# rodluger/starry_process

Hardware: AMD Instinct MI355X
Metric: log_likelihood evals/sec (ydeg=15, K=1000) (higher is better)
Workload: dtype f64

## Files before the change

starry_process_amd/csrc/sp_cov.h:

```cpp
#ifndef SP_COV_H
#define SP_COV_H

#include "sp_internal.h"

__device__ __forceinline__ int star_nobs(const sp_star &st, int K) {
  return (st.nobs > 0 && st.nobs < K) ? st.nobs : K;
}

__device__ __forceinline__ double temporal_factor(int kind, double ti, double tj,
                                                  double tau) {
#pragma clang fp contract(off)
  if (kind == SP_TEMPORAL_NONE) return 1.0;
  const double dt = fabs(ti - tj);
  if (kind == SP_TEMPORAL_MATERN32) {
    const double x = 1.7320508075688772 * dt / tau;
    return (1.0 + x) * exp(-x);
  }
  return exp(-(dt * dt) / (2.0 * tau));
}

__device__ __forceinline__ double temporal_dfactor_dtau(int kind, double ti, double tj,
                                                        double tau) {
  if (kind == SP_TEMPORAL_NONE) return 0.0;
  const double dt = fabs(ti - tj);
  if (kind == SP_TEMPORAL_MATERN32) {
    const double x = 1.7320508075688772 * dt / tau;
    return x * x / tau * exp(-x);
  }
  return (dt * dt) / (2.0 * tau * tau) * exp(-(dt * dt) / (2.0 * tau));
}

template <int CTRL>
__device__ __forceinline__ double dpp_move(double v) {
  const int lo = __builtin_amdgcn_mov_dpp(__double2loint(v), CTRL, 0xf, 0xf, true);
  const int hi = __builtin_amdgcn_mov_dpp(__double2hiint(v), CTRL, 0xf, 0xf, true);
  return __hiloint2double(hi, lo);
}
template <int N>
__device__ __forceinline__ void row16_sum(double (&x)[N]) {
#pragma unroll
  for (int k = 0; k < N; ++k) x[k] += dpp_move<0xB1>(x[k]);
#pragma unroll
  for (int k = 0; k < N; ++k) x[k] += dpp_move<0x4E>(x[k]);
#pragma unroll
  for (int k = 0; k < N; ++k) x[k] += dpp_move<0x141>(x[k]);
#pragma unroll
  for (int k = 0; k < N; ++k) x[k] += dpp_move<0x140>(x[k]);
}

typedef double dd2 __attribute__((ext_vector_type(2)));

struct SplineGen {
  const double *tab;
  int np2;
  double dx, inv_dx;
  int covpts;
  __device__ __forceinline__ double operator()(double thi, double thj) const {
#pragma clang fp contract(off)
    const double x = fabs(thi - thj);
    const double q = x * inv_dx;
    int idx = (int)q;
    double x0 = q - (double)idx;
    if (fabs(x0 - 0.5) > 0.5 - 1.0e-9) {
      idx = (int)floor(x / dx);
      x0 = q - (double)idx;
    }
    idx = idx > covpts ? covpts : idx;
    typedef const __attribute__((address_space(3))) dd2 *lds_dd2;
    const unsigned a1 = (unsigned)(size_t)(const __attribute__((address_space(3))) double *)tab + ((unsigned)idx << 4);
    const dd2 c01 = *(lds_dd2)(size_t)a1;
    const dd2 c23 = *(lds_dd2)(size_t)(a1 + 8u * (unsigned)np2);
    return __builtin_fma(x0, __builtin_fma(x0, __builtin_fma(x0, c23.y, c23.x), c01.y), c01.x);
  }
  template <int N>
  __device__ __forceinline__ void many(const double (&thi)[N], const double (&thj)[N], double (&out)[N]) const {
#pragma clang fp contract(off)
    double x0[N];
    int idx[N];
    bool odd = false;
#pragma unroll
    for (int e = 0; e < N; ++e) {
      const double q = fabs(thi[e] - thj[e]) * inv_dx;
      idx[e] = (int)q;
      x0[e] = q - (double)idx[e];
      odd |= fabs(x0[e] - 0.5) > 0.5 - 1.0e-9;
    }
    if (__builtin_expect(odd, 0)) {
#pragma unroll
      for (int e = 0; e < N; ++e)
        if (fabs(x0[e] - 0.5) > 0.5 - 1.0e-9) {
          const double x = fabs(thi[e] - thj[e]);
          idx[e] = (int)floor(x / dx);
          x0[e] = x * inv_dx - (double)idx[e];
        }
    }
    dd2 c01[N], c23[N];
    typedef const __attribute__((address_space(3))) dd2 *lds_dd2;
    const unsigned base = (unsigned)(size_t)(const __attribute__((address_space(3))) double *)tab;
    const unsigned off2 = 8u * (unsigned)np2;
#pragma unroll
    for (int e = 0; e < N; ++e) {
      const int k = idx[e] > covpts ? covpts : idx[e];
      const unsigned a1 = base + ((unsigned)k << 4);
      c01[e] = *(lds_dd2)(size_t)a1;
      c23[e] = *(lds_dd2)(size_t)(a1 + off2);
    }
#pragma unroll
    for (int e = 0; e < N; ++e)
      out[e] = __builtin_fma(x0[e], __builtin_fma(x0[e], __builtin_fma(x0[e], c23[e].y, c23[e].x), c01[e].y), c01[e].x);
  }
};


__device__ __forceinline__ void spline_table_to_lds(const double *__restrict__ src, double *stage, int np, int tid) {
  const int n2 = 2 * np;
  dd2 v[4];
#pragma unroll
  for (int c = 0; c < 4; ++c) {
    const int e = tid + 256 * c;
    v[c] = e < n2 ? *reinterpret_cast<const dd2 *>(src + 2 * e) : dd2{0.0, 0.0};
  }
#pragma unroll
  for (int c = 0; c < 4; ++c) {
    const int e = tid + 256 * c;
    if (e < n2) *reinterpret_cast<dd2 *>(stage + 2 * e) = v[c];
  }
  for (int e = tid + 1024; e < n2; e += 256)
    *reinterpret_cast<dd2 *>(stage + 2 * e) = *reinterpret_cast<const dd2 *>(src + 2 * e);
}


#ifndef SP_LAZY_BATCH
#define SP_LAZY_BATCH 8
#endif
template <int MA, typename V4>
__device__ __forceinline__ void lazy_cov_tiles(const LazyCov &z, int star, const int (&ri)[MA][4],
                                               const int (&cj)[4], V4 (&out)[MA][4], double *stage) {
  const sp_star st = z.stars[star];
  const int nobs = star_nobs(st, z.K), np = z.covpts + 4;
  const double *th = z.theta + (size_t)star * z.K, *tt = z.t + (size_t)star * z.K;
  const bool tk = z.temporal != SP_TEMPORAL_NONE;
#ifdef SP_LAZY_NO_SEP
  const bool sep = false;
#else
  const bool sep = z.temporal == SP_TEMPORAL_MATERN32 && z.inorder && z.inorder[star] != 0.0;
#endif
  double thi[MA][4], ti[MA][4], thj[4], tj[4];
#pragma unroll
  for (int k = 0; k < 4; ++k) {
    const bool oj = cj[k] < nobs;
    thj[k] = oj ? th[cj[k]] : 0.0;
    tj[k] = (oj && tk) ? tt[cj[k]] : 0.0;
#pragma unroll
    for (int m = 0; m < MA; ++m) {
      const bool oi = ri[m][k] < nobs;
      thi[m][k] = oi ? th[ri[m][k]] : 0.0;
      ti[m][k] = (oi && tk) ? tt[ri[m][k]] : 0.0;
    }
  }
  const int c0 = cj[0] & ~63;
  const double tb = sep ? tt[c0 < nobs ? c0 : nobs - 1] : 0.0;
  spline_table_to_lds(z.ptab + (size_t)star * 4 * np, stage, np, threadIdx.x);
  __syncthreads();
  SplineGen g{stage, 2 * np, 6.283185307179586 / z.covpts,
              1.0 / (6.283185307179586 / z.covpts), z.covpts};
  const double cm = sep ? 1.7320508075688772 / st.tau : 0.0;
  double fc[4] = {1.0, 1.0, 1.0, 1.0};
  bool fok[4] = {false, false, false, false};
  if (sep) {
#pragma unroll
    for (int n = 0; n < 4; ++n) {
      const double a = cm * (tj[n] - tb);
      fok[n] = a < 600.0 && a >= 0.0;
      fc[n] = exp(fok[n] ? a : 0.0);
    }
  }
#pragma unroll
  for (int m = 0; m < MA; ++m) {
    double er[4] = {1.0, 1.0, 1.0, 1.0};
    if (sep) {
#pragma unroll
      for (int r = 0; r < 4; ++r) er[r] = exp(-(cm * (ti[m][r] - tb)));
    }
#pragma unroll
    for (int n0 = 0; n0 < 4; n0 += SP_LAZY_BATCH / 4) {
      double a[SP_LAZY_BATCH], b[SP_LAZY_BATCH], v[SP_LAZY_BATCH];
#pragma unroll
      for (int e = 0; e < SP_LAZY_BATCH; ++e) {
        a[e] = thi[m][e & 3];
        b[e] = thj[n0 + (e >> 2)];
      }
      g.many<SP_LAZY_BATCH>(a, b, v);
#pragma unroll
      for (int e = 0; e < SP_LAZY_BATCH; ++e) {
        const int n = n0 + (e >> 2), r = e & 3;
        double w = 0.0;
        if (ri[m][r] < nobs && cj[n] < nobs) {
#pragma clang fp contract(off)
          if (sep && fok[n]) {
            const double x = cm * (ti[m][r] - tj[n]);
            w = v[e] * ((1.0 + x) * (er[r] * fc[n]));
          } else {
            w = v[e] * temporal_factor(z.temporal, ti[m][r], tj[n], st.tau);
          }
        }
        out[m][n][r] = w;
      }
    }
    if (z.rid) {
#pragma unroll
      for (int r = 0; r < 4; ++r) {
        const int mr = ri[m][r] - z.K;
        if (mr < 0 || mr >= z.nrid) continue;
        const double *src = z.rid + ((size_t)star * (z.nrid + 1) + mr) * z.K;
        double x[4];
#pragma unroll
        for (int n = 0; n < 4; ++n) x[n] = src[cj[n] < z.K ? cj[n] : z.K - 1];
#pragma unroll
        for (int n = 0; n < 4; ++n) out[m][n][r] = cj[n] < z.K ? x[n] : 0.0;
      }
    }
  }
  __syncthreads();
}

template <typename V4>
__device__ __forceinline__ void lazy_diag_block(const LazyCov &z, int star, const SplineGen &g, const sp_star &st,
                                                int nobs, const int (&ri)[4], int cj, V4 &out) {
  const double *th = z.theta + (size_t)star * z.K, *tt = z.t + (size_t)star * z.K;
  const double *rb = z.rid + (size_t)star * (z.nrid + 1) * z.K;
  const bool tk = z.temporal != SP_TEMPORAL_NONE;
  const int cc = cj < z.K ? cj : z.K - 1;
  const double thj = th[cc], tj = tk ? tt[cc] : 0.0;
  double thi[4], ti[4], dd[4], rv[4];
#pragma unroll
  for (int r = 0; r < 4; ++r) {
    const int rc = ri[r] < z.K ? ri[r] : z.K - 1;
    thi[r] = th[rc];
    ti[r] = tk ? tt[rc] : 0.0;
    dd[r] = rb[(size_t)z.nrid * z.K + rc];
    const int m = ri[r] - z.K;
    rv[r] = rb[(size_t)((m >= 0 && m < z.nrid) ? m : 0) * z.K + cc];
  }
#pragma unroll
  for (int r = 0; r < 4; ++r) {
    const int m = ri[r] - z.K;
    double v;
    if (ri[r] < nobs && cj < nobs) {
#pragma clang fp contract(off)
      v = g(thi[r], thj) * temporal_factor(z.temporal, ti[r], tj, st.tau);
      if (ri[r] == cj) v += dd[r];
    } else if (m >= 0 && m < z.nrid && cj < z.K) {
      v = rv[r];
    } else {
      v = ri[r] == cj ? 1.0 : 0.0;
    }
    out[r] = v;
  }
}

#ifndef SP_LAZY_ROW_BATCH
#define SP_LAZY_ROW_BATCH 0
#endif
template <int ROWB, typename V4>
__device__ __forceinline__ void lazy_cov_row(const LazyCov &z, int star, int ri, int c0, V4 (&out)[4],
                                             double *stage, int tid) {
  const sp_star st = z.stars[star];
  const int nobs = star_nobs(st, z.K), np = z.covpts + 4;
  const double *th = z.theta + (size_t)star * z.K;
  const bool oi = ri < nobs;
  const double thi = oi ? th[ri] : 0.0;
  double *s_thj = stage + 4 * np;
  {
    const double *src = z.ptab + (size_t)star * 4 * np;
    const int n2 = 2 * np, cbase = c0 & ~63;
    dd2 v[3];
#pragma unroll
    for (int c = 0; c < 3; ++c) {
      const int e = tid + 256 * c;
      v[c] = e < n2 ? *reinterpret_cast<const dd2 *>(src + 2 * e) : dd2{0.0, 0.0};
    }
    const double tj = (tid < 64 && cbase + tid < nobs) ? th[cbase + tid] : 0.0;
#pragma unroll
    for (int c = 0; c < 3; ++c) {
      const int e = tid + 256 * c;
      if (e < n2) *reinterpret_cast<dd2 *>(stage + 2 * e) = v[c];
    }
    for (int e = tid + 768; e < n2; e += 256)
      *reinterpret_cast<dd2 *>(stage + 2 * e) = *reinterpret_cast<const dd2 *>(src + 2 * e);
    if (tid < 64) s_thj[tid] = tj;
  }
  __syncthreads();
  SplineGen g{stage, 2 * np, 6.283185307179586 / z.covpts,
              1.0 / (6.283185307179586 / z.covpts), z.covpts};
  const int cl = c0 & 63;
  if constexpr (ROWB == 2) {
#pragma unroll
  for (int m = 0; m < 4; ++m) {
    V4 o;
#pragma unroll
    for (int half = 0; half < 2; ++half) {
      const dd2 tt = *reinterpret_cast<const dd2 *>(s_thj + cl + 16 * m + 2 * half);
      const double a[2] = {thi, thi}, b[2] = {tt.x, tt.y};
      double v[2];
      g.many<2>(a, b, v);
      o[2 * half] = (oi && c0 + 16 * m + 2 * half < nobs) ? v[0] : 0.0;
      o[2 * half + 1] = (oi && c0 + 16 * m + 2 * half + 1 < nobs) ? v[1] : 0.0;
      __builtin_amdgcn_sched_barrier(0);
    }
    out[m] = o;
  }
  } else if constexpr (ROWB == 0) {
#pragma unroll
  for (int m = 0; m < 4; ++m) {
    const dd2 t01 = *reinterpret_cast<const dd2 *>(s_thj + cl + 16 * m), t23 = *reinterpret_cast<const dd2 *>(s_thj + cl + 16 * m + 2);
    const double thj[4] = {t01.x, t01.y, t23.x, t23.y};
    V4 o;
#pragma unroll
    for (int r = 0; r < 4; ++r) o[r] = (oi && c0 + 16 * m + r < nobs) ? g(thi, thj[r]) : 0.0;
    out[m] = o;
  }
  } else {
#pragma unroll
  for (int m0 = 0; m0 < 4; m0 += ROWB / 4) {
    double a[ROWB], b[ROWB], v[ROWB];
#pragma unroll
    for (int h = 0; h < ROWB / 4; ++h) {
      const dd2 t01 = *reinterpret_cast<const dd2 *>(s_thj + cl + 16 * (m0 + h));
      const dd2 t23 = *reinterpret_cast<const dd2 *>(s_thj + cl + 16 * (m0 + h) + 2);
      a[4 * h] = a[4 * h + 1] = a[4 * h + 2] = a[4 * h + 3] = thi;
      b[4 * h] = t01.x;
      b[4 * h + 1] = t01.y;
      b[4 * h + 2] = t23.x;
      b[4 * h + 3] = t23.y;
    }
    g.many<ROWB>(a, b, v);
#pragma unroll
    for (int h = 0; h < ROWB / 4; ++h) {
      V4 o;
#pragma unroll
      for (int r = 0; r < 4; ++r) o[r] = (oi && c0 + 16 * (m0 + h) + r < nobs) ? v[4 * h + r] : 0.0;
      out[m0 + h] = o;
    }
    __builtin_amdgcn_sched_barrier(0);
  }
  }
  if (z.rid && !oi) {
    const int mr = ri - z.K;
    if (mr >= 0 && mr < z.nrid) {
      const double *src = z.rid + ((size_t)star * (z.nrid + 1) + mr) * z.K;
      double x[16];
#pragma unroll
      for (int e = 0; e < 16; ++e) {
        const int c = c0 + 16 * (e >> 2) + (e & 3);
        x[e] = src[c < z.K ? c : z.K - 1];
      }
#pragma unroll
      for (int m = 0; m < 4; ++m) {
        V4 o;
#pragma unroll
        for (int r = 0; r < 4; ++r) o[r] = c0 + 16 * m + r < z.K ? x[4 * m + r] : 0.0;
        out[m] = o;
      }
    }
  }
  __syncthreads();
}

#endif
```

starry_process_amd/csrc/sp_gemm.hip:

```cpp
#include <cstdlib>

#include <type_traits>

#include "sp_internal.h"
#include "sp_tile.h"
#include "sp_cov.h"
#include "sp_mm.h"
#include "sp_stage.h"
#include "sp_paneldiag.h"

typedef double d2 __attribute__((ext_vector_type(2)));

#define GT SP_GT

namespace {

__global__ __launch_bounds__(256) void gemm_nt_kernel(
    const double *A, long lda, long strideA, const double *__restrict__ B, long ldb, long strideB,
    double *C, long ldc, long strideC, int Mrows, int Nrows, int Kd, double alpha, int beta,
    int lower_only, int batch, int ntn, int ntiles, const int32_t *__restrict__ bsel, int nsel) {
  constexpr int BK = 32, LDW = BK + 1;
  __shared__ __attribute__((aligned(16))) double smem[2 * GT * LDW];
  double *sA = smem, *sB = smem + GT * LDW;
  int mtx, tile;
  if (!sp_xcd_decode(blockIdx.x, batch, ntiles, mtx, tile)) return;
  int ti, tj;
  if (lower_only) {
    ti = (int)((sqrt(8.0 * tile + 1.0) - 1.0) * 0.5);
    while (ti * (ti + 1) / 2 > tile) --ti;
    while ((ti + 1) * (ti + 2) / 2 <= tile) ++ti;
    tj = tile - ti * (ti + 1) / 2;
  } else {
    ti = tile / ntn;
    tj = tile % ntn;
  }
  const int row0 = ti * GT, col0 = tj * GT;
  const double *Ab = A + (size_t)mtx * strideA;
  int bm = mtx;
  if (bsel) {
    bm = bsel[mtx];
    if (bm < 0 || bm >= nsel) bm = 0;
  }
  const double *Bb = B + (size_t)bm * strideB;
  double *Cb = C + (size_t)mtx * strideC;
  const int lane = threadIdx.x & 63, wave = threadIdx.x >> 6;
  const int fr = lane & 15, fk = lane >> 4;
  d4 acc[4];
#pragma unroll
  for (int n = 0; n < 4; ++n) acc[n] = d4{0.0, 0.0, 0.0, 0.0};
  const bool full = row0 + GT <= Mrows && col0 + GT <= Nrows;
  if (beta) {
#pragma unroll
    for (int n = 0; n < 4; ++n)
#pragma unroll
      for (int r = 0; r < 4; ++r) {
        const int gi = row0 + 16 * wave + fk + 4 * r, gj = col0 + 16 * n + fr;
        if (full || (gi < Mrows && gj < Nrows)) acc[n][r] = Cb[(size_t)gi * ldc + gj];
      }
  }
  const bool vecA = ((lda & 1) == 0) && ((reinterpret_cast<uintptr_t>(Ab) & 15) == 0);
  const bool vecB = ((ldb & 1) == 0) && ((reinterpret_cast<uintptr_t>(Bb) & 15) == 0);
  PanelRegs<BK> ra, rb;
  if (Kd > 0) {
    stage_load<BK>(Ab, lda, row0, Mrows, 0, Kd, vecA, ra);
    stage_load<BK>(Bb, ldb, col0, Nrows, 0, Kd, vecB, rb);
  }
  for (int k0 = 0; k0 < Kd; k0 += BK) {
    stage_store<BK>(ra, alpha, sA);
    stage_store<BK>(rb, 1.0, sB);
    __syncthreads();
    if (k0 + BK < Kd) {
      stage_load<BK>(Ab, lda, row0, Mrows, k0 + BK, Kd, vecA, ra);
      stage_load<BK>(Bb, ldb, col0, Nrows, k0 + BK, Kd, vecB, rb);
    }
    const double *pa = sA + (16 * wave + fr) * LDW + fk;
    const double *pb = sB + fr * LDW + fk;
#pragma unroll
    for (int kk = 0; kk < BK; kk += 4) {
      const double a = pa[kk];
      acc[0] = __builtin_amdgcn_mfma_f64_16x16x4f64(a, pb[kk], acc[0], 0, 0, 0);
      acc[1] = __builtin_amdgcn_mfma_f64_16x16x4f64(a, pb[16 * LDW + kk], acc[1], 0, 0, 0);
      acc[2] = __builtin_amdgcn_mfma_f64_16x16x4f64(a, pb[32 * LDW + kk], acc[2], 0, 0, 0);
      acc[3] = __builtin_amdgcn_mfma_f64_16x16x4f64(a, pb[48 * LDW + kk], acc[3], 0, 0, 0);
    }
    __syncthreads();
  }
#pragma unroll
  for (int n = 0; n < 4; ++n)
#pragma unroll
    for (int r = 0; r < 4; ++r) {
      const int gi = row0 + 16 * wave + fk + 4 * r, gj = col0 + 16 * n + fr;
      if (full || (gi < Mrows && gj < Nrows)) Cb[(size_t)gi * ldc + gj] = acc[n][r];
    }
}

}

namespace {
#ifdef SP_MM_STAMPS
__device__ long long sp_mm_dbg[8 * 4096];
#endif
#ifndef SP_MM_WAVES
#define SP_MM_WAVES 1
#endif
#ifndef SP_MM_SYRK_NS
#define SP_MM_SYRK_NS 6
#endif
template <class Core, bool SGN, bool SEL = false>
__global__ __launch_bounds__(256, SP_MM_WAVES) void mm_nt_kernel(
    const double *__restrict__ A, long lda, long strideA, const double *__restrict__ B, long ldb,
    long strideB, double *__restrict__ C, long ldc, long strideC, int Kd, double alpha, int beta,
    int lower_only, int batch, int ntn, int ntiles, int skip00, LazyCov lz, DiagFuse df,
    const int32_t *__restrict__ bsel, int nsel) {
  constexpr int TM = Core::TM_, TN = Core::TN_;
  static_assert(Core::LDS_DOUBLES >= SP_DIAG_LDS_DOUBLES, "the tile-(0,0) workgroup factors a pivot block in this LDS");
  __shared__ __attribute__((aligned(16))) double lds[Core::LDS_DOUBLES];
#ifdef SP_MM_STAMPS
  const long long wall_begin = wall_clock64(), cyc_begin = __builtin_readcyclecounter();
#endif
  int mtx, tile;
  if (!sp_xcd_decode(blockIdx.x, batch, ntiles, mtx, tile)) return;
  int ti, tj;
  if (lower_only) {
    ti = (int)((sqrt(8.0 * tile + 1.0) - 1.0) * 0.5);
    while (ti * (ti + 1) / 2 > tile) --ti;
    while ((ti + 1) * (ti + 2) / 2 <= tile) ++ti;
    tj = tile - ti * (ti + 1) / 2;
  } else {
    ti = tile / ntn;
    tj = tile % ntn;
  }
  const int tj_limit = skip00 >> 8;
  int k_first = (skip00 & 2) ? ti * TM : 0;
  if (df.tri0 >= 0 && TM == 64) {
    const int r = 64 * (df.j + ti) - df.tri0, first = r > 0 ? r / 64 - df.s0 : 0;
    if (first > 0) k_first = 64 * first < Kd ? 64 * first : Kd;
  }
  if (tj_limit && tj >= tj_limit) return;
  if ((skip00 & 1) && lower_only && ti == 0 && tj == 0) {
    if (df.sys) {
      __builtin_amdgcn_s_setprio(3);
      panel_diag_item(df.sys + (size_t)mtx * df.stride, df.ld, df.j, df.nact,
                      df.img + (size_t)mtx * df.lts + sp_img_off(df.j),
                      df.info ? df.info + mtx : nullptr, lds, threadIdx.x);
    }
    return;
  }
  const double *Ab = A + (size_t)mtx * strideA + (size_t)ti * TM * lda;
  int bm = mtx;
  if constexpr (SEL) {
    bm = bsel[mtx];
    if (bm < 0 || bm >= nsel) bm = 0;
  }
  const double *Bb = B + (size_t)bm * strideB + (size_t)tj * TN * ldb;
  double *Cb = C + (size_t)mtx * strideC + (size_t)ti * TM * ldc + (size_t)tj * TN;
  Core mm;
  mm.init(Ab, lda, Bb, ldb);
  if constexpr (SGN && Core::MA == 1 && Core::NA == 4 && TM == 64 && TN == 64) {
    if ((skip00 & 4) && lower_only && ti == tj) {
      const bool dform = beta && lz.theta && (lz.dlazy & 2);
      const int lane = threadIdx.x & 63;
      sp_star dst{};
      int dnobs = 0;
      if (dform) {
        dst = lz.stars[mtx];
        dnobs = star_nobs(dst, lz.K);
        spline_table_to_lds(lz.ptab + (size_t)mtx * 4 * (lz.covpts + 4), lds, lz.covpts + 4, threadIdx.x);
        __syncthreads();
      }
      const SplineGen dg{lds, 2 * (lz.covpts + 4), 6.283185307179586 / lz.covpts, 1.0 / (6.283185307179586 / lz.covpts),
                         lz.covpts};
      if (!dform) mm.prologue(lds, k_first, Kd);
      auto run = [&](auto wtag) {
        constexpr int W = decltype(wtag)::value;
        using D = typename Core::template SymDeal<W>;
        mm_d4 a3[3];
#pragma unroll
        for (int b = 0; b < 3; ++b) {
          mm_d4 c = mm_d4{0.0, 0.0, 0.0, 0.0};
          if (b < D::NB && dform) {
            int ri[4];
#pragma unroll
            for (int r = 0; r < 4; ++r) ri[r] = 64 * (lz.tr0 + ti) + 16 * D::brow(b) + (lane >> 4) + 4 * r;
            lazy_diag_block(lz, mtx, dg, dst, dnobs, ri, 64 * (lz.tc0 + tj) + 16 * D::bcol(b) + (lane & 15), c);
          } else if (b < D::NB && beta) {
#pragma unroll
            for (int r = 0; r < 4; ++r)
              c[r] = Cb[(size_t)(16 * D::brow(b) + (lane >> 4) + 4 * r) * ldc + 16 * D::bcol(b) + (lane & 15)];
          }
          a3[b] = alpha < 0.0 ? -c : c;
        }
        if (dform) {
          __syncthreads();
          mm.prologue(lds, k_first, Kd);
        }
        mm.template sym_loop<W>(lds, k_first, Kd, a3);
#pragma unroll
        for (int b = 0; b < D::NB; ++b)
#pragma unroll
          for (int r = 0; r < 4; ++r)
            Cb[(size_t)(16 * D::brow(b) + (lane >> 4) + 4 * r) * ldc + 16 * D::bcol(b) + (lane & 15)] =
                alpha < 0.0 ? -a3[b][r] : a3[b][r];
      };
      switch (threadIdx.x >> 6) {
        case 0: run(std::integral_constant<int, 0>{}); break;
        case 1: run(std::integral_constant<int, 1>{}); break;
        case 2: run(std::integral_constant<int, 2>{}); break;
        default: run(std::integral_constant<int, 3>{}); break;
      }
      return;
    }
  }
  mm_d4 acc[Core::MA][Core::NA], cin[SGN ? 1 : Core::MA][SGN ? 1 : Core::NA];
  constexpr bool CAN_LAZY = Core::MA == 1 && Core::NA == 4 && TM == 64 && TN == 64;
  const bool lazy = CAN_LAZY && beta && lz.theta && lz.tr0 + ti > lz.tc0 + tj && lz.tc0 + tj > 0 &&
                    lz.tr0 + ti < lz.nfull;
  mm_d4 cz1[1][4];
  mm_d4 (&cz)[4] = cz1[0];
  if (!lazy) mm.prologue(lds, k_first, Kd);
  if (lazy) {
    int ri[1][4], cj[4];
#pragma unroll
    for (int k = 0; k < 4; ++k) {
      ri[0][k] = 64 * (lz.tr0 + ti) + mm.acc_row(0, k);
      cj[k] = 64 * (lz.tc0 + tj) + mm.acc_col(k < Core::NA ? k : 0);
    }
    lazy_cov_tiles<1>(lz, mtx, ri, cj, cz1, lds);
    mm.prologue(lds, k_first, Kd);
  }
#pragma unroll
  for (int m = 0; m < Core::MA; ++m)
#pragma unroll
    for (int n = 0; n < Core::NA; ++n) {
      mm_d4 c = mm_d4{0.0, 0.0, 0.0, 0.0};
      if (lazy) {
        c = cz[n & 3];
      } else if (beta) {
#pragma unroll
        for (int r = 0; r < 4; ++r) c[r] = Cb[(size_t)mm.acc_row(m, r) * ldc + mm.acc_col(n)];
      }
      if (SGN) {
        acc[m][n] = alpha < 0.0 ? -c : c;
      } else {
        acc[m][n] = mm_d4{0.0, 0.0, 0.0, 0.0};
        cin[m][n] = c;
      }
    }
#ifdef SP_MM_STAMPS
  const long long cyc_loop = __builtin_readcyclecounter();
#endif
  mm.loop(lds, k_first, Kd, acc);
#ifdef SP_MM_STAMPS
  const long long cyc_store = __builtin_readcyclecounter();
#endif
#pragma unroll
  for (int m = 0; m < Core::MA; ++m)
#pragma unroll
    for (int n = 0; n < Core::NA; ++n)
#pragma unroll
      for (int r = 0; r < 4; ++r) {
        double v;
        if (SGN)
          v = alpha < 0.0 ? -acc[m][n][r] : acc[m][n][r];
        else
          v = fma(alpha, acc[m][n][r], cin[m][n][r]);
        Cb[(size_t)mm.acc_row(m, r) * ldc + mm.acc_col(n)] = v;
      }
#ifdef SP_MM_STAMPS
  if (threadIdx.x == 0 && lower_only && df.sys && blockIdx.x < 4096) {
    long long *o = sp_mm_dbg + 8 * blockIdx.x;
    o[0] = (long long)mtx * 4096 + tile; o[1] = lazy; o[2] = wall_begin; o[3] = wall_clock64();
    o[4] = cyc_loop - cyc_begin; o[5] = cyc_store - cyc_loop; o[6] = __builtin_readcyclecounter() - cyc_store;
    o[7] = ((__builtin_amdgcn_s_getreg(20 | (0 << 6) | (31 << 11)) & 15u) << 8) | ((__builtin_amdgcn_s_getreg(4 | (0 << 6) | (31 << 11)) >> 8) & 255u);
  }
#endif
}


using Syrk128Core = MM2<128, 64, 8, 4, 4>;
#ifndef SP_SYRK128_WGS
#define SP_SYRK128_WGS 1
#endif
__global__ __launch_bounds__(256, SP_SYRK128_WGS) void syrk128_kernel(const double *__restrict__ X, long ld, long stride,
                                                      double *__restrict__ T, int Kd, int batch, int nb, int ntiles,
                                                      LazyCov lz, DiagFuse df) {
  using Core = Syrk128Core;
  static_assert(Core::LDS_DOUBLES >= SP_DIAG_LDS_DOUBLES, "the last workgroup of a star factors a pivot block in this LDS");
  static_assert(Core::MA == 2 && Core::NA == 4, "a wavefront = 32 rows of one block row");
  __shared__ __attribute__((aligned(16))) double lds[Core::LDS_DOUBLES];
  int mtx, tile;
  if (!sp_xcd_decode(blockIdx.x, batch, ntiles, mtx, tile)) return;
  if (tile == 0) {
    if (df.sys) {
      __builtin_amdgcn_s_setprio(3);
      panel_diag_item(df.sys + (size_t)mtx * df.stride, df.ld, df.j, df.nact,
                      df.img + (size_t)mtx * df.lts + sp_img_off(df.j), df.info ? df.info + mtx : nullptr, lds, threadIdx.x);
    }
    return;
  }
  tile -= 1;
  const int o = nb & 1;
  int I = (int)((sqrt((double)((o + 1) * (o + 1) + 4 * tile)) - (o + 1)) * 0.5);
  while (I * I + I * (o + 1) > tile) --I;
  while ((I + 1) * (I + 1) + (I + 1) * (o + 1) <= tile) ++I;
  const int J = tile - (I * I + I * (o + 1)), R0 = o + 2 * I;
  const double *Xb = X + (size_t)mtx * stride;
  const double *Ab = Xb + (size_t)R0 * 64 * ld, *Bb = Xb + (size_t)J * 64 * ld;
  double *Cb = T + (size_t)mtx * stride + (size_t)R0 * 64 * ld + (size_t)J * 64;
  Core mm;
  mm.init(Ab, ld, Bb, ld);
  const int R = R0 + (mm.acc_row(0, 0) >> 6);
  const bool want = R >= J && !(R == 0 && J == 0);
  const auto is_lazy = [&](int Rb) {
    return lz.theta && lz.tr0 + Rb > lz.tc0 + J && lz.tc0 + J > 0 && lz.tr0 + Rb < lz.nfull;
  };
  const bool any_lazy = is_lazy(R0) || is_lazy(R0 + 1), my_lazy = is_lazy(R);
  mm_d4 acc[Core::MA][Core::NA];
  if (any_lazy) {
    int ri[Core::MA][4], cj[4];
#pragma unroll
    for (int k = 0; k < 4; ++k) {
      cj[k] = 64 * (lz.tc0 + J) + mm.acc_col(k);
#pragma unroll
      for (int m = 0; m < Core::MA; ++m) ri[m][k] = 64 * (lz.tr0 + R0) + mm.acc_row(m, k);
    }
    lazy_cov_tiles<Core::MA>(lz, mtx, ri, cj, acc, lds);
  }
  mm.prologue(lds, 0, Kd);
#pragma unroll
  for (int m = 0; m < Core::MA; ++m)
#pragma unroll
    for (int n = 0; n < Core::NA; ++n) {
      mm_d4 c = mm_d4{0.0, 0.0, 0.0, 0.0};
      if (any_lazy && my_lazy) {
        c = acc[m][n];
      } else if (want) {
#pragma unroll
        for (int r = 0; r < 4; ++r) c[r] = Cb[(size_t)mm.acc_row(m, r) * ld + mm.acc_col(n)];
      }
      acc[m][n] = -c;
    }
  mm.loop(lds, 0, Kd, acc);
  if (!want) return;
#pragma unroll
  for (int m = 0; m < Core::MA; ++m)
#pragma unroll
    for (int n = 0; n < Core::NA; ++n)
#pragma unroll
      for (int r = 0; r < 4; ++r) Cb[(size_t)mm.acc_row(m, r) * ld + mm.acc_col(n)] = -acc[m][n][r];
}

template <class Core>
int mm_launch(const double *A, long lda, long strideA, const double *B, long ldb, long strideB,
              double *C, long ldc, long strideC, int Mrows, int Nrows, int Kd, double alpha, int beta,
              int lower_only, int batch, hipStream_t st, int skip00, const LazyCov *lazy = nullptr,
              const DiagFuse *dfp = nullptr, const int32_t *bsel = nullptr, int nsel = 0) {
  const LazyCov lz = lazy ? *lazy : LazyCov{};
  const DiagFuse df = dfp ? *dfp : DiagFuse{nullptr, 0, 0, 0, 0, nullptr, 0, nullptr, -1, 0};
  const int ntm = Mrows / Core::TM_, ntn = Nrows / Core::TN_;
  const int ntiles = lower_only ? ntm * (ntm + 1) / 2 : ntm * ntn;
  const long nblk = sp_xcd_grid(batch, ntiles);
  if (nblk > 0x7fffffffL) return SP_ERR_INVALID;
  if (bsel) {
    if (alpha != 1.0 || lazy || dfp) return SP_ERR_INVALID;
    hipLaunchKernelGGL((mm_nt_kernel<Core, true, true>), dim3((unsigned)nblk), dim3(256), 0, st,
                       A, lda, strideA, B, ldb, strideB, C, ldc, strideC, Kd, alpha, beta, lower_only,
                       batch, ntn, ntiles, skip00, lz, df, bsel, nsel);
  } else if (alpha == 1.0 || alpha == -1.0)
    hipLaunchKernelGGL((mm_nt_kernel<Core, true>), dim3((unsigned)nblk), dim3(256), 0, st,
                       A, lda, strideA, B, ldb, strideB, C, ldc, strideC, Kd, alpha, beta, lower_only,
                       batch, ntn, ntiles, skip00, lz, df, (const int32_t *)nullptr, 0);
  else
    hipLaunchKernelGGL((mm_nt_kernel<Core, false>), dim3((unsigned)nblk), dim3(256), 0, st,
                       A, lda, strideA, B, ldb, strideB, C, ldc, strideC, Kd, alpha, beta, lower_only,
                       batch, ntn, ntiles, skip00, lz, df, (const int32_t *)nullptr, 0);
  SP_LAUNCH_CHECK();
  return SP_OK;
}
}

#ifdef SP_MM_STAMPS
extern "C" int sp_debug_mm_stamps(long long *out, int n) {
  return (int)hipMemcpyFromSymbol(out, HIP_SYMBOL(sp_mm_dbg), sizeof(long long) * n);
}
#endif

static int launch_gemm(const double *A, long lda, long strideA, const double *B, long ldb,
                       long strideB, double *C, long ldc, long strideC, int Mrows, int Nrows,
                       int Kd, double alpha, int beta, int lower_only, int batch, hipStream_t st,
                       int skip00 = 0, const LazyCov *lazy = nullptr, const int32_t *bsel = nullptr, int nsel = 0) {
  if (bsel && (nsel < 1 || skip00 || (lazy && lazy->theta))) return SP_ERR_INVALID;
  if (Mrows <= 0 || Nrows <= 0 || batch <= 0) return SP_OK;
  if (Kd < 0) return SP_ERR_INVALID;
  const int ntm = (Mrows + GT - 1) / GT, ntn = (Nrows + GT - 1) / GT;
  if (lower_only && ntm != ntn) return SP_ERR_INVALID;
  const int ntiles = lower_only ? ntm * (ntm + 1) / 2 : ntm * ntn;
  const long nblk = sp_xcd_grid(batch, ntiles);
  if (nblk > 0x7fffffffL) return SP_ERR_INVALID;
  const bool fast = (Mrows % GT) == 0 && (Nrows % GT) == 0 && (Kd % 32) == 0 && Kd > 0 &&
                    ((lda | ldb) & 1) == 0 && (strideA & 1) == 0 && (strideB & 1) == 0 &&
                    ((reinterpret_cast<uintptr_t>(A) | reinterpret_cast<uintptr_t>(B)) & 15) == 0;
  if (lazy && lazy->theta) {
    if (!fast) return SP_ERR_INVALID;
    return mm_launch<MM2<64, 64, 8, 6, 4>>(A, lda, strideA, B, ldb, strideB, C, ldc, strideC, Mrows, Nrows,
                                           Kd, alpha, beta, lower_only, batch, st, skip00, lazy);
  }
  if (fast) {
#ifdef SP_MM_TILE_PROBE
    static const int probe = getenv("SP_MM_TILE") ? atoi(getenv("SP_MM_TILE")) : 0;
    if (!bsel && !lower_only && probe == 1 && (Mrows % 128) == 0)
      return mm_launch<MM2<128, 64, 8, 4, 4>>(A, lda, strideA, B, ldb, strideB, C, ldc, strideC, Mrows, Nrows, Kd, alpha,
                                              beta, lower_only, batch, st, skip00);
    if (!bsel && !lower_only && probe == 2 && (Mrows % 128) == 0)
      return mm_launch<MM2<128, 64, 8, 5, 4>>(A, lda, strideA, B, ldb, strideB, C, ldc, strideC, Mrows, Nrows, Kd, alpha,
                                              beta, lower_only, batch, st, skip00);
    if (!bsel && !lower_only && probe == 3 && (Mrows % 128) == 0)
      return mm_launch<MM2<128, 64, 16, 3, 4>>(A, lda, strideA, B, ldb, strideB, C, ldc, strideC, Mrows, Nrows, Kd, alpha,
                                               beta, lower_only, batch, st, skip00);
    if (!bsel && !lower_only && probe == 4)
      return mm_launch<MM2<64, 64, 8, 6, 4>>(A, lda, strideA, B, ldb, strideB, C, ldc, strideC, Mrows, Nrows, Kd, alpha,
                                             beta, lower_only, batch, st, skip00);
#endif
    if (!lower_only && (Mrows % 128) == 0 && (Nrows % 128) == 0)
      return mm_launch<MM2<128, 128, 8, 4, 2>>(A, lda, strideA, B, ldb, strideB, C, ldc, strideC, Mrows,
                                               Nrows, Kd, alpha, beta, lower_only, batch, st, skip00, nullptr, nullptr,
                                               bsel, nsel);
    return mm_launch<MM2<64, 64, 8, 6, 4>>(A, lda, strideA, B, ldb, strideB, C, ldc, strideC, Mrows, Nrows,
                                           Kd, alpha, beta, lower_only, batch, st, skip00, nullptr, nullptr, bsel, nsel);
  }
  if (skip00) return SP_ERR_INVALID;
  hipLaunchKernelGGL(gemm_nt_kernel, dim3((unsigned)nblk), dim3(256), 0, st, A, lda, strideA, B, ldb,
                     strideB, C, ldc, strideC, Mrows, Nrows, Kd, alpha, beta, lower_only, batch, ntn, ntiles, bsel, nsel);
  SP_LAUNCH_CHECK();
  return SP_OK;
}

static int g_syrk128_from = -1;
static int syrk128_from() {
  if (g_syrk128_from < 0) {
    const char *e = getenv("SP_SYRK128_FROM");
    g_syrk128_from = e ? atoi(e) : 17;
    if (g_syrk128_from < 0) g_syrk128_from = 0;
  }
  return g_syrk128_from;
}
extern "C" int sp_debug_set_syrk128_from(int blocks) {
  g_syrk128_from = blocks < 0 ? -1 : blocks;
  return SP_OK;
}

static int g_syrk_symdiag = -1;
static int syrk_symdiag() {
  if (g_syrk_symdiag < 0) {
    const char *e = getenv("SP_SYRK_SYMDIAG");
    g_syrk_symdiag = (e && atoi(e) == 0) ? 0 : 1;
  }
  return g_syrk_symdiag;
}
int sp_syrk_can_form_diag(int nb) {
  const int big_from = syrk128_from();
  return (syrk_symdiag() && !(big_from > 0 && nb >= big_from)) ? 1 : 0;
}
extern "C" int sp_debug_set_syrk_symdiag(int on) {
  g_syrk_symdiag = on < 0 ? -1 : (on ? 1 : 0);
  return SP_OK;
}

int sp_launch_syrk_diag(const double *X, long ld, long stride, double *T, int n, int kd, int batch,
                        hipStream_t st, const LazyCov *lazy, const DiagFuse *df, int tj_limit) {
  if (n <= 0 || batch <= 0) return SP_OK;
  if ((n % GT) || (kd % 16) || kd <= 0 || (ld & 1) || (stride & 1) ||
      ((reinterpret_cast<uintptr_t>(X) | reinterpret_cast<uintptr_t>(T)) & 15))
    return SP_ERR_INVALID;
  const int big_from = syrk128_from();
  const int nb = n / GT;
  if (big_from > 0 && nb >= big_from && tj_limit == 0 && (!df || df->tri0 < 0) && (kd % 16) == 0) {
    const int o = nb & 1, nrt = (nb - o) / 2, ntiles = nrt * nrt + nrt * (o + 1) + 1;
    const long nblk = sp_xcd_grid(batch, ntiles);
    if (nblk > 0x7fffffffL) return SP_ERR_INVALID;
    const DiagFuse d = df ? *df : DiagFuse{nullptr, 0, 0, 0, 0, nullptr, 0, nullptr, -1, 0};
    const LazyCov lzv = (lazy && lazy->theta) ? *lazy : LazyCov{};
    hipLaunchKernelGGL(syrk128_kernel, dim3((unsigned)nblk), dim3(256), 0, st, X, ld, stride, T, kd, batch, nb, ntiles, lzv, d);
    SP_LAUNCH_CHECK();
    return SP_OK;
  }
  const int symdiag = syrk_symdiag() ? 4 : 0;
  return mm_launch<MM2<64, 64, 8, SP_MM_SYRK_NS, 4>>(X, ld, stride, X, ld, stride, T, ld, stride, n, n, kd, -1.0, 1, 1,
                                         batch, st, 1 | symdiag | (tj_limit > 0 ? tj_limit << 8 : 0),
                                         (lazy && lazy->theta) ? lazy : nullptr, df);
}

int sp_launch_gemm_nt(const double *A, long lda, long strideA, const double *B, long ldb,
                      long strideB, double *C, long ldc, long strideC, int Mrows, int Nrows,
                      int Kd, double alpha, int beta, int lower_only, int batch,
                      hipStream_t st, int skip_tile00, const LazyCov *lazy, const int32_t *bsel, int nsel) {
  return launch_gemm(A, lda, strideA, B, ldb, strideB, C, ldc, strideC, Mrows, Nrows, Kd,
                     alpha, beta, lower_only, batch, st, skip_tile00, lazy, bsel, nsel);
}
```

starry_process_amd/csrc/sp_mm.h:

```cpp
#ifndef SP_MM_H
#define SP_MM_H

#include <hip/hip_runtime.h>

typedef double mm_d4 __attribute__((ext_vector_type(4)));

template <int N>
__device__ __forceinline__ void mm_wait_vmcnt() {
  if constexpr (N == 0) asm volatile("s_waitcnt vmcnt(0)" ::: "memory");
  else if constexpr (N == 1) asm volatile("s_waitcnt vmcnt(1)" ::: "memory");
  else if constexpr (N == 2) asm volatile("s_waitcnt vmcnt(2)" ::: "memory");
  else if constexpr (N == 3) asm volatile("s_waitcnt vmcnt(3)" ::: "memory");
  else if constexpr (N == 4) asm volatile("s_waitcnt vmcnt(4)" ::: "memory");
  else if constexpr (N == 6) asm volatile("s_waitcnt vmcnt(6)" ::: "memory");
  else if constexpr (N == 8) asm volatile("s_waitcnt vmcnt(8)" ::: "memory");
  else if constexpr (N == 9) asm volatile("s_waitcnt vmcnt(9)" ::: "memory");
  else if constexpr (N == 10) asm volatile("s_waitcnt vmcnt(10)" ::: "memory");
  else if constexpr (N == 14) asm volatile("s_waitcnt vmcnt(14)" ::: "memory");
  else if constexpr (N == 12) asm volatile("s_waitcnt vmcnt(12)" ::: "memory");
  else if constexpr (N == 16) asm volatile("s_waitcnt vmcnt(16)" ::: "memory");
  else if constexpr (N == 18) asm volatile("s_waitcnt vmcnt(18)" ::: "memory");
  else if constexpr (N == 24) asm volatile("s_waitcnt vmcnt(24)" ::: "memory");
  else static_assert(N < 0, "add the immediate to mm_wait_vmcnt");
}

template <int TM, int TN, int BK, int NS, int WR>
struct MM2 {
  static constexpr int TM_ = TM, TN_ = TN;
  static constexpr int WC = 4 / WR;
  static constexpr int MA = TM / (16 * WR), NA = TN / (16 * WC);
  static constexpr int G = BK / 2, RPI = 64 / G, RPB = 32 / BK;
  static constexpr int IA = TM / RPI, IB = TN / RPI, LA = IA / 4, LB = IB / 4, LPW = LA + LB;
  static constexpr int STAGE_A = TM * BK, STAGE_B = TN * BK, STAGE = STAGE_A + STAGE_B;
  static constexpr int LDS_DOUBLES = NS * STAGE;
  static constexpr int NC = BK / 8;
  static_assert(BK == 8 || BK == 16 || BK == 32, "slice depth");
  static_assert(IA % 4 == 0 && IB % 4 == 0, "a slice must split evenly over four wavefronts");
  static_assert(NS >= 3, "one slice in registers, one landing, one being issued");
  typedef double v2 __attribute__((ext_vector_type(2)));
  struct Frags {
    v2 a[NC][MA], b[NC][NA];
  };
  __device__ static __forceinline__ int swz(int row) {
    const int fr = row & 15;
#ifdef SP_MM_OLD_SWZ
    return (fr / RPB) & (G - 1);
#endif
    return ((fr / RPB) ^ (((fr >> 2) ^ (fr >> 3)) & 1)) & (G - 1);
  }

  const double *srcA[LA > 0 ? LA : 1];
  const double *srcB[LB > 0 ? LB : 1];
  int rdA, rdB, fsw, q, wave;

  __device__ __forceinline__ void init(const double *A, long lda, const double *B, long ldb) {
    const int lane = threadIdx.x & 63;
    wave = threadIdx.x >> 6;
    const int r = lane / G, p = lane % G;
#pragma unroll
    for (int i = 0; i < LA; ++i) {
      const int row = (wave + 4 * i) * RPI + r;
      srcA[i] = A + (size_t)row * lda + 2 * (p ^ swz(row));
    }
#pragma unroll
    for (int i = 0; i < LB; ++i) {
      const int row = (wave + 4 * i) * RPI + r;
      srcB[i] = B + (size_t)row * ldb + 2 * (p ^ swz(row));
    }
    const int wr = wave / WC, wc = wave % WC, fr = lane & 15;
    rdA = (wr * (TM / WR) + fr) * BK;
    rdB = STAGE_A + (wc * (TN / WC) + fr) * BK;
    fsw = swz(fr);
    q = lane >> 4;
  }
  __device__ __forceinline__ void issue(double *lds, int st, int k0) const {
    double *base = lds + st * STAGE;
#pragma unroll
    for (int i = 0; i < LA; ++i)
      __builtin_amdgcn_global_load_lds(
          (const __attribute__((address_space(1))) void *)(srcA[i] + k0),
          (__attribute__((address_space(3))) void *)(base + (wave + 4 * i) * 128), 16, 0, 0);
#pragma unroll
    for (int i = 0; i < LB; ++i)
      __builtin_amdgcn_global_load_lds(
          (const __attribute__((address_space(1))) void *)(srcB[i] + k0),
          (__attribute__((address_space(3))) void *)(base + STAGE_A + (wave + 4 * i) * 128), 16, 0, 0);
  }
  __device__ __forceinline__ void fetch(const double *lds, int st, Frags &f) const {
    const double *base = lds + st * STAGE;
#pragma unroll
    for (int c = 0; c < NC; ++c) {
      const int goff = 2 * ((4 * c + q) ^ fsw);
#pragma unroll
      for (int m = 0; m < MA; ++m) f.a[c][m] = *reinterpret_cast<const v2 *>(base + rdA + m * 16 * BK + goff);
#pragma unroll
      for (int n = 0; n < NA; ++n) f.b[c][n] = *reinterpret_cast<const v2 *>(base + rdB + n * 16 * BK + goff);
    }
  }
  __device__ __forceinline__ void mul(const Frags &f, mm_d4 (&acc)[MA][NA]) const {
#pragma unroll
    for (int c = 0; c < NC; ++c)
#pragma unroll
      for (int h = 0; h < 2; ++h)
#pragma unroll
        for (int m = 0; m < MA; ++m)
#pragma unroll
          for (int n = 0; n < NA; ++n)
            acc[m][n] = __builtin_amdgcn_mfma_f64_16x16x4f64(h ? f.a[c][m].y : f.a[c][m].x,
                                                            h ? f.b[c][n].y : f.b[c][n].x, acc[m][n], 0, 0, 0);
  }
  __device__ __forceinline__ void mul_fetch(const Frags &cur, Frags &nxt, const double *lds, int st,
                                            mm_d4 (&acc)[MA][NA]) const {
    const double *base = lds + st * STAGE;
    constexpr int NR = NC * (MA + NA);
    int issued = 0;
#pragma unroll
    for (int c = 0; c < NC; ++c)
#pragma unroll
      for (int h = 0; h < 2; ++h)
#pragma unroll
        for (int m = 0; m < MA; ++m)
#pragma unroll
          for (int n = 0; n < NA; ++n) {
            acc[m][n] = __builtin_amdgcn_mfma_f64_16x16x4f64(h ? cur.a[c][m].y : cur.a[c][m].x,
                                                            h ? cur.b[c][n].y : cur.b[c][n].x, acc[m][n], 0, 0, 0);
            __builtin_amdgcn_sched_group_barrier(0x008, 1, 0);
            if (issued < NR) {
              const int rc = issued / (MA + NA), ri = issued % (MA + NA);
              const int goff = 2 * ((4 * rc + q) ^ fsw);
              if (ri < MA)
                nxt.a[rc][ri] = *reinterpret_cast<const v2 *>(base + rdA + ri * 16 * BK + goff);
              else
                nxt.b[rc][ri - MA] = *reinterpret_cast<const v2 *>(base + rdB + (ri - MA) * 16 * BK + goff);
              __builtin_amdgcn_sched_group_barrier(0x100, 1, 0);
              ++issued;
            }
          }
    static_assert(NR <= NC * 2 * MA * NA, "more fragment reads than MFMAs to hide them behind");
  }
  __device__ __forceinline__ void prologue(double *lds, int k_begin, int k_end) const {
    const int nsl = (k_end - k_begin) / BK;
#pragma unroll
    for (int p = 0; p < NS - 1; ++p)
      if (p < nsl) issue(lds, p, k_begin + p * BK);
  }
  __device__ __forceinline__ void loop(double *lds, int k_begin, int k_end, mm_d4 (&acc)[MA][NA],
                                       int fence = 1 << 30) const {
    const int nsl = (k_end - k_begin) / BK;
    if (nsl <= 0) return;
    Frags f0, f1;
    if (nsl >= NS - 1) mm_wait_vmcnt<(NS - 2) * LPW>(); else mm_wait_vmcnt<0>();
    __builtin_amdgcn_s_barrier();
    fetch(lds, 0, f0);
    int st1 = 1 % NS;
    int stn = NS - 1;
    for (int s = 0; s < nsl; s += 2) {
      if (s + NS - 1 < nsl && s + NS - 1 != fence) mm_wait_vmcnt<(NS - 3) * LPW>(); else mm_wait_vmcnt<0>();
      __builtin_amdgcn_s_barrier();
      if (s + NS - 1 < nsl) issue(lds, stn, k_begin + (s + NS - 1) * BK);
      mul_fetch(f0, f1, lds, st1, acc);
      st1 = st1 + 1 == NS ? 0 : st1 + 1;
      stn = stn + 1 == NS ? 0 : stn + 1;
      if (s + 2 < nsl) {
        if (s + NS < nsl && s + NS != fence) mm_wait_vmcnt<(NS - 3) * LPW>(); else mm_wait_vmcnt<0>();
        __builtin_amdgcn_s_barrier();
        if (s + NS < nsl) issue(lds, stn, k_begin + (s + NS) * BK);
      }
      mul_fetch(f1, f0, lds, st1, acc);
      st1 = st1 + 1 == NS ? 0 : st1 + 1;
      stn = stn + 1 == NS ? 0 : stn + 1;
    }
    __builtin_amdgcn_s_barrier();
  }
  template <int W>
  struct SymDeal {
    static constexpr int NB = W < 2 ? 3 : 2;
    static constexpr int NF = W == 1 ? 4 : (W == 3 ? 2 : 3);
    __device__ static constexpr int frow(int f) {
      return W == 0 ? (f == 0 ? 0 : f == 1 ? 1 : 3) : W == 1 ? f : W == 2 ? f : (f == 0 ? 2 : 3);
    }
    __device__ static constexpr int brow(int b) {
      return W == 0 ? (b == 0 ? 0 : 3) : W == 1 ? (b < 2 ? 1 : 3) : W == 2 ? 2 : (b == 0 ? 2 : 3);
    }
    __device__ static constexpr int bcol(int b) {
      return W == 0 ? (b == 0 ? 0 : b - 1) : W == 1 ? b : W == 2 ? b : (b == 0 ? 2 : 3);
    }
    __device__ static constexpr int fidx(int row) {
      return W == 0 ? (row == 3 ? 2 : row) : W == 1 ? row : W == 2 ? row : row - 2;
    }
  };
  template <int W>
  struct SymFrags {
    v2 f[NC][SymDeal<W>::NF];
  };
  template <int W>
  __device__ __forceinline__ void sym_fetch(const double *lds, int st, SymFrags<W> &fr) const {
    const double *base = lds + st * STAGE + (threadIdx.x & 15) * BK;
#pragma unroll
    for (int c = 0; c < NC; ++c) {
      const int goff = 2 * ((4 * c + q) ^ fsw);
#pragma unroll
      for (int i = 0; i < SymDeal<W>::NF; ++i)
        fr.f[c][i] = *reinterpret_cast<const v2 *>(base + SymDeal<W>::frow(i) * 16 * BK + goff);
    }
  }
  template <int W>
  __device__ __forceinline__ void sym_mul_fetch(const SymFrags<W> &cur, SymFrags<W> &nxt, const double *lds, int st,
                                                mm_d4 (&acc)[3]) const {
    using D = SymDeal<W>;
    const double *base = lds + st * STAGE + (threadIdx.x & 15) * BK;
    constexpr int NR = NC * D::NF;
    int issued = 0;
#pragma unroll
    for (int c = 0; c < NC; ++c)
#pragma unroll
      for (int h = 0; h < 2; ++h)
#pragma unroll
        for (int b = 0; b < D::NB; ++b) {
          const v2 a = cur.f[c][D::fidx(D::brow(b))], bb = cur.f[c][D::fidx(D::bcol(b))];
          acc[b] = __builtin_amdgcn_mfma_f64_16x16x4f64(h ? a.y : a.x, h ? bb.y : bb.x, acc[b], 0, 0, 0);
          __builtin_amdgcn_sched_group_barrier(0x008, 1, 0);
          if (issued < NR) {
            const int rc = issued / D::NF, ri = issued % D::NF;
            const int goff = 2 * ((4 * rc + q) ^ fsw);
            nxt.f[rc][ri] = *reinterpret_cast<const v2 *>(base + D::frow(ri) * 16 * BK + goff);
            __builtin_amdgcn_sched_group_barrier(0x100, 1, 0);
            ++issued;
          }
        }
    static_assert(NR <= NC * 2 * D::NB, "more fragment reads than MFMAs to hide them behind");
  }
  template <int W>
  __device__ __forceinline__ void sym_loop(double *lds, int k_begin, int k_end, mm_d4 (&acc)[3]) const {
    const int nsl = (k_end - k_begin) / BK;
    if (nsl <= 0) return;
    SymFrags<W> f0, f1;
    if (nsl >= NS - 1) mm_wait_vmcnt<(NS - 2) * LPW>(); else mm_wait_vmcnt<0>();
    __builtin_amdgcn_s_barrier();
    sym_fetch<W>(lds, 0, f0);
    int st1 = 1 % NS, stn = NS - 1;
    for (int s = 0; s < nsl; s += 2) {
      if (s + NS - 1 < nsl) mm_wait_vmcnt<(NS - 3) * LPW>(); else mm_wait_vmcnt<0>();
      __builtin_amdgcn_s_barrier();
      if (s + NS - 1 < nsl) issue(lds, stn, k_begin + (s + NS - 1) * BK);
      sym_mul_fetch<W>(f0, f1, lds, st1, acc);
      st1 = st1 + 1 == NS ? 0 : st1 + 1;
      stn = stn + 1 == NS ? 0 : stn + 1;
      if (s + 2 < nsl) {
        if (s + NS < nsl) mm_wait_vmcnt<(NS - 3) * LPW>(); else mm_wait_vmcnt<0>();
        __builtin_amdgcn_s_barrier();
        if (s + NS < nsl) issue(lds, stn, k_begin + (s + NS) * BK);
      }
      sym_mul_fetch<W>(f1, f0, lds, st1, acc);
      st1 = st1 + 1 == NS ? 0 : st1 + 1;
      stn = stn + 1 == NS ? 0 : stn + 1;
    }
    __builtin_amdgcn_s_barrier();
  }

  __device__ __forceinline__ int acc_row(int m, int r) const {
    const int lane = threadIdx.x & 63;
    return (wave / WC) * (TM / WR) + 16 * m + (lane >> 4) + 4 * r;
  }
  __device__ __forceinline__ int acc_col(int n) const {
    const int lane = threadIdx.x & 63;
    return (wave % WC) * (TN / WC) + 16 * n + (lane & 15);
  }
};

#endif
```

Measured before the change: 106,600.

## Switch SYRK core to 2x2 accumulator layout with three workgroups per CU

The SYRK trailing-update launch moves from a 1x4 accumulator arrangement (MA=1, NA=4) to a 2x2 one (MA=2, NA=2). To support this, the lazy covariance tile generator and the diagonal-tile path are generalised to arbitrary MA/NA, and the symmetric tile dealing across waves is remapped. Launch bounds ask for three workgroups per CU for the 2x2 core, trading register budget for occupancy and changing per-wave fragment reuse. This risks register spills and a different LDS fragment-reuse pattern.

```diff
diff --git a/starry_process_amd/csrc/sp_cov.h b/starry_process_amd/csrc/sp_cov.h
--- a/starry_process_amd/csrc/sp_cov.h
+++ b/starry_process_amd/csrc/sp_cov.h
@@ -133,9 +133,10 @@
 #ifndef SP_LAZY_BATCH
 #define SP_LAZY_BATCH 8
 #endif
-template <int MA, typename V4>
+template <int MA, int NA = 4, typename V4>
 __device__ __forceinline__ void lazy_cov_tiles(const LazyCov &z, int star, const int (&ri)[MA][4],
-                                               const int (&cj)[4], V4 (&out)[MA][4], double *stage) {
+                                               const int (&cj)[NA], V4 (&out)[MA][NA], double *stage) {
+  static_assert(4 * NA % SP_LAZY_BATCH == 0, "whole batches");
   const sp_star st = z.stars[star];
   const int nobs = star_nobs(st, z.K), np = z.covpts + 4;
   const double *th = z.theta + (size_t)star * z.K, *tt = z.t + (size_t)star * z.K;
@@ -145,12 +146,15 @@
 #else
   const bool sep = z.temporal == SP_TEMPORAL_MATERN32 && z.inorder && z.inorder[star] != 0.0;
 #endif
-  double thi[MA][4], ti[MA][4], thj[4], tj[4];
-#pragma unroll
-  for (int k = 0; k < 4; ++k) {
+  double thi[MA][4], ti[MA][4], thj[NA], tj[NA];
+#pragma unroll
+  for (int k = 0; k < NA; ++k) {
     const bool oj = cj[k] < nobs;
     thj[k] = oj ? th[cj[k]] : 0.0;
     tj[k] = (oj && tk) ? tt[cj[k]] : 0.0;
+  }
+#pragma unroll
+  for (int k = 0; k < 4; ++k) {
 #pragma unroll
     for (int m = 0; m < MA; ++m) {
       const bool oi = ri[m][k] < nobs;
@@ -165,11 +169,16 @@
   SplineGen g{stage, 2 * np, 6.283185307179586 / z.covpts,
               1.0 / (6.283185307179586 / z.covpts), z.covpts};
   const double cm = sep ? 1.7320508075688772 / st.tau : 0.0;
-  double fc[4] = {1.0, 1.0, 1.0, 1.0};
-  bool fok[4] = {false, false, false, false};
+  double fc[NA];
+  bool fok[NA];
+#pragma unroll
+  for (int n = 0; n < NA; ++n) {
+    fc[n] = 1.0;
+    fok[n] = false;
+  }
   if (sep) {
 #pragma unroll
-    for (int n = 0; n < 4; ++n) {
+    for (int n = 0; n < NA; ++n) {
       const double a = cm * (tj[n] - tb);
       fok[n] = a < 600.0 && a >= 0.0;
       fc[n] = exp(fok[n] ? a : 0.0);
@@ -183,7 +192,7 @@
       for (int r = 0; r < 4; ++r) er[r] = exp(-(cm * (ti[m][r] - tb)));
     }
 #pragma unroll
-    for (int n0 = 0; n0 < 4; n0 += SP_LAZY_BATCH / 4) {
+    for (int n0 = 0; n0 < NA; n0 += SP_LAZY_BATCH / 4) {
       double a[SP_LAZY_BATCH], b[SP_LAZY_BATCH], v[SP_LAZY_BATCH];
 #pragma unroll
       for (int e = 0; e < SP_LAZY_BATCH; ++e) {
@@ -213,11 +222,11 @@
         const int mr = ri[m][r] - z.K;
         if (mr < 0 || mr >= z.nrid) continue;
         const double *src = z.rid + ((size_t)star * (z.nrid + 1) + mr) * z.K;
-        double x[4];
-#pragma unroll
-        for (int n = 0; n < 4; ++n) x[n] = src[cj[n] < z.K ? cj[n] : z.K - 1];
-#pragma unroll
-        for (int n = 0; n < 4; ++n) out[m][n][r] = cj[n] < z.K ? x[n] : 0.0;
+        double x[NA];
+#pragma unroll
+        for (int n = 0; n < NA; ++n) x[n] = src[cj[n] < z.K ? cj[n] : z.K - 1];
+#pragma unroll
+        for (int n = 0; n < NA; ++n) out[m][n][r] = cj[n] < z.K ? x[n] : 0.0;
       }
     }
   }
diff --git a/starry_process_amd/csrc/sp_gemm.hip b/starry_process_amd/csrc/sp_gemm.hip
--- a/starry_process_amd/csrc/sp_gemm.hip
+++ b/starry_process_amd/csrc/sp_gemm.hip
@@ -106,8 +106,10 @@
 #ifndef SP_MM_SYRK_NS
 #define SP_MM_SYRK_NS 6
 #endif
+template <class Core>
+constexpr int mm_wgs_per_cu = (Core::MA == 2 && Core::NA == 2 && SP_MM_WAVES < 3) ? 3 : SP_MM_WAVES;
 template <class Core, bool SGN, bool SEL = false>
-__global__ __launch_bounds__(256, SP_MM_WAVES) void mm_nt_kernel(
+__global__ __launch_bounds__(256, mm_wgs_per_cu<Core>) void mm_nt_kernel(
     const double *__restrict__ A, long lda, long strideA, const double *__restrict__ B, long ldb,
     long strideB, double *__restrict__ C, long ldc, long strideC, int Kd, double alpha, int beta,
     int lower_only, int batch, int ntn, int ntiles, int skip00, LazyCov lz, DiagFuse df,
@@ -156,7 +158,7 @@
   double *Cb = C + (size_t)mtx * strideC + (size_t)ti * TM * ldc + (size_t)tj * TN;
   Core mm;
   mm.init(Ab, lda, Bb, ldb);
-  if constexpr (SGN && Core::MA == 1 && Core::NA == 4 && TM == 64 && TN == 64) {
+  if constexpr (SGN && TM == 64 && TN == 64) {
     if ((skip00 & 4) && lower_only && ti == tj) {
       const bool dform = beta && lz.theta && (lz.dlazy & 2);
       const int lane = threadIdx.x & 63;
@@ -212,20 +214,20 @@
     }
   }
   mm_d4 acc[Core::MA][Core::NA], cin[SGN ? 1 : Core::MA][SGN ? 1 : Core::NA];
-  constexpr bool CAN_LAZY = Core::MA == 1 && Core::NA == 4 && TM == 64 && TN == 64;
+  constexpr bool CAN_LAZY = TM == 64 && TN == 64;
   const bool lazy = CAN_LAZY && beta && lz.theta && lz.tr0 + ti > lz.tc0 + tj && lz.tc0 + tj > 0 &&
                     lz.tr0 + ti < lz.nfull;
-  mm_d4 cz1[1][4];
-  mm_d4 (&cz)[4] = cz1[0];
+  mm_d4 cz[Core::MA][Core::NA];
   if (!lazy) mm.prologue(lds, k_first, Kd);
   if (lazy) {
-    int ri[1][4], cj[4];
-#pragma unroll
-    for (int k = 0; k < 4; ++k) {
-      ri[0][k] = 64 * (lz.tr0 + ti) + mm.acc_row(0, k);
-      cj[k] = 64 * (lz.tc0 + tj) + mm.acc_col(k < Core::NA ? k : 0);
-    }
-    lazy_cov_tiles<1>(lz, mtx, ri, cj, cz1, lds);
+    int ri[Core::MA][4], cj[Core::NA];
+#pragma unroll
+    for (int m = 0; m < Core::MA; ++m)
+#pragma unroll
+      for (int k = 0; k < 4; ++k) ri[m][k] = 64 * (lz.tr0 + ti) + mm.acc_row(m, k);
+#pragma unroll
+    for (int n = 0; n < Core::NA; ++n) cj[n] = 64 * (lz.tc0 + tj) + mm.acc_col(n);
+    lazy_cov_tiles<Core::MA, Core::NA>(lz, mtx, ri, cj, cz, lds);
     mm.prologue(lds, k_first, Kd);
   }
 #pragma unroll
@@ -234,7 +236,7 @@
     for (int n = 0; n < Core::NA; ++n) {
       mm_d4 c = mm_d4{0.0, 0.0, 0.0, 0.0};
       if (lazy) {
-        c = cz[n & 3];
+        c = cz[m][n];
       } else if (beta) {
 #pragma unroll
         for (int r = 0; r < 4; ++r) c[r] = Cb[(size_t)mm.acc_row(m, r) * ldc + mm.acc_col(n)];
@@ -485,7 +487,7 @@
     return SP_OK;
   }
   const int symdiag = syrk_symdiag() ? 4 : 0;
-  return mm_launch<MM2<64, 64, 8, SP_MM_SYRK_NS, 4>>(X, ld, stride, X, ld, stride, T, ld, stride, n, n, kd, -1.0, 1, 1,
+  return mm_launch<MM2<64, 64, 8, SP_MM_SYRK_NS, 2>>(X, ld, stride, X, ld, stride, T, ld, stride, n, n, kd, -1.0, 1, 1,
                                          batch, st, 1 | symdiag | (tj_limit > 0 ? tj_limit << 8 : 0),
                                          (lazy && lazy->theta) ? lazy : nullptr, df);
 }
diff --git a/starry_process_amd/csrc/sp_mm.h b/starry_process_amd/csrc/sp_mm.h
--- a/starry_process_amd/csrc/sp_mm.h
+++ b/starry_process_amd/csrc/sp_mm.h
@@ -175,18 +175,18 @@
   template <int W>
   struct SymDeal {
     static constexpr int NB = W < 2 ? 3 : 2;
-    static constexpr int NF = W == 1 ? 4 : (W == 3 ? 2 : 3);
+    static constexpr int NF = (W == 0 || W == 3) ? 2 : 3;
     __device__ static constexpr int frow(int f) {
-      return W == 0 ? (f == 0 ? 0 : f == 1 ? 1 : 3) : W == 1 ? f : W == 2 ? f : (f == 0 ? 2 : 3);
+      return W == 0 ? f : W == 1 ? f : W == 2 ? (f == 2 ? 3 : f) : 2 + f;
     }
     __device__ static constexpr int brow(int b) {
-      return W == 0 ? (b == 0 ? 0 : 3) : W == 1 ? (b < 2 ? 1 : 3) : W == 2 ? 2 : (b == 0 ? 2 : 3);
+      return W == 0 ? (b == 0 ? 0 : 1) : W == 1 ? 2 : 3;
     }
     __device__ static constexpr int bcol(int b) {
-      return W == 0 ? (b == 0 ? 0 : b - 1) : W == 1 ? b : W == 2 ? b : (b == 0 ? 2 : 3);
+      return W == 0 ? (b == 0 ? 0 : b - 1) : W == 1 ? b : W == 2 ? b : 2 + b;
     }
     __device__ static constexpr int fidx(int row) {
-      return W == 0 ? (row == 3 ? 2 : row) : W == 1 ? row : W == 2 ? row : row - 2;
+      return W == 0 ? row : W == 1 ? row : W == 2 ? (row == 3 ? 2 : row) : row - 2;
     }
   };
   template <int W>
```

Result: no change. 106,400 (-0.2%).
